# Sweethyh/GaussianImage_plus

Hardware: AMD Instinct MI355X
Metric: training iters/sec (fwd+bwd rasterize) at N Gaussians, 768x512 (higher is better)
Workload: dtype f32

## Files before the change

gaussianimage_plus_amd/csrc/gi2d_fused_core.h:

```cpp
#pragma once
#include <cstdint>

#include <hip/hip_runtime.h>

#ifdef GI2D_FUSED_TRACE
namespace gi2d {
__device__ unsigned long long *g_fused_trace = nullptr;
}
#define GI2D_TRACE_AT(wg, i)                                                                        \
    do {                                                                                            \
        if (threadIdx.x == 0 && g_fused_trace) g_fused_trace[(wg) * 16 + (i)] = wall_clock64();     \
    } while (0)
#define GI2D_TRACE(i) GI2D_TRACE_AT(tile, i)
#define GI2D_TRACE_VALUE(i, v)                                                        \
    do {                                                                              \
        if (threadIdx.x == 0 && g_fused_trace) g_fused_trace[tile * 16 + (i)] = (v);  \
    } while (0)
#define GI2D_BWD_TRACE(i) GI2D_TRACE_AT(blockIdx.x, i)
#define GI2D_HEAD_TRACE(i) GI2D_TRACE_AT(tile, i)
#else
#define GI2D_TRACE(i) \
    do {              \
    } while (0)
#define GI2D_TRACE_VALUE(i, v) \
    do {                       \
    } while (0)
#endif

#include "gi2d_fast_internal.h"

namespace gi2d {

#ifndef GI2D_FUSED_OCC
#define GI2D_FUSED_OCC 6
#endif

#ifndef GI2D_SMALL_CAP
#define GI2D_SMALL_CAP 128
#endif
template <int CAP>
struct FusedLdsT {
    static constexpr int PSTR = 9;
    static constexpr bool HAS_FIDX = false;
    static constexpr bool HAS_RAW = false;
    static constexpr int PART_ROWS = GI2D_BWD_PART_ROWS;
    static constexpr int LISTLEN = CAP + 8;
    static constexpr int IDS = CAP == GI2D_TILE_LIST_CAP ? GI2D_FAST_C : CAP;
    float4 gA[CAP + 1];
    float4 gB[CAP + 1];
    float2 gC[CAP + 2];
    unsigned cullw[CAP];
    float sse_w[4];
    int scan_w[8];
    int grp[32];
    union {
        struct {
            int ids[IDS];
        };
        struct {
            unsigned char lists[4][2 * LISTLEN];
            float4 pairbuf[GI2D_FWD_PAIRBUF];
        };
        struct {
            float4 pix[2 * GI2D_BWD_PIXRECS];
            unsigned short span[CAP];
            unsigned short item[8 * CAP];
            float part[GI2D_BWD_PART_ROWS * PSTR];
            int wsum[8];
            int n_items;
        };
        struct {
            char fwd_reach[sizeof(unsigned char) * 4 * 2 * LISTLEN + sizeof(float4) * GI2D_FWD_PAIRBUF];
            int slot[CAP];
        };
    };
    __device__ __forceinline__ void set_box(int, unsigned) {}
    __device__ __forceinline__ unsigned box_of(int k) const { return cullw[k] >> 8; }
};
typedef FusedLdsT<GI2D_TILE_LIST_CAP> FusedLds;
typedef FusedLdsT<GI2D_SMALL_CAP> FusedLdsSmall;
#ifndef GI2D_SMALL_OCC
#define GI2D_SMALL_OCC 8
#endif

static_assert(GI2D_FUSED_OCC < 6 || sizeof(FusedLds) <= 26624,
              "FusedLds: the sixth workgroup per CU needs <= 26 KB (see GI2D_FUSED_OCC)");
static_assert(sizeof(FusedLdsSmall) <= 160 * 1024 / GI2D_SMALL_OCC - 512, "FusedLdsSmall: eight workgroups per CU need <= 19.5 KB");
static_assert(offsetof(FusedLds, slot) >= offsetof(FusedLds, part) &&
                  offsetof(FusedLds, slot) + sizeof(int) * GI2D_TILE_LIST_CAP <= offsetof(FusedLds, wsum),
              "FusedLds: the partial-row codes must overlay the hand-off buffer only");
static_assert(offsetof(FusedLdsSmall, slot) >= offsetof(FusedLdsSmall, part) &&
                  offsetof(FusedLdsSmall, slot) + sizeof(int) * GI2D_SMALL_CAP <= offsetof(FusedLdsSmall, wsum),
              "FusedLdsSmall: the partial-row codes must overlay the hand-off buffer only");

template <int MODE, int CAP = GI2D_TILE_LIST_CAP, int FWD_UNROLL = GI2D_FWD_UNROLL, bool INBOX = false, bool WT = false>
__device__ __forceinline__ void fused_tile(
    FusedLdsT<CAP> &sm, int tile, int tiles_x, int tiles_y, int img_w, int img_h, const float4 *__restrict__ recs,
    int32_t *__restrict__ lists, int2 *__restrict__ tile_bins,
    float4 *__restrict__ partial_g, float4 *__restrict__ partial_big, int32_t *__restrict__ status,
    float *__restrict__ out_img, const float *__restrict__ vsrc, float grad_scale, float *__restrict__ tile_sse,
    const HeadRow head_row, const Inbox &ib) {
    const int tx = tile % tiles_x, ty = tile / tiles_x;
    const int pool_rows = tiles_x * tiles_y * GI2D_TILE_LIST_CAP;
    static_assert(CAP <= GI2D_TILE_LIST_CAP, "at most the reference's 256 entries of a tile are rasterized");
    const int tid = threadIdx.x, lane = tid & 63, wv = tid >> 6;
    const int lx = fwd_lane_col(tid), ly = tid >> 4;
    const int j = tx * GI2D_TILE + lx, i = ty * GI2D_TILE + ly;
    const bool inside = (i < img_h) && (j < img_w);
    const size_t pix = (size_t)i * img_w + j;

    GI2D_TRACE(0);
    float p0 = 0.f, p1 = 0.f, p2 = 0.f;
    if (inside) {
        p0 = vsrc[3 * pix];
        p1 = vsrc[3 * pix + 1];
        p2 = vsrc[3 * pix + 2];
    }

    if (tid == 0) {
        sm.gA[CAP] = make_float4(0.f, 0.f, 0.f, 0.f);
        sm.gB[CAP] = make_float4(0.f, 0.f, 0.f, 0.f);
        sm.gC[CAP] = make_float2(0.f, 0.f);
    }
    GI2D_TRACE_VALUE(1, (unsigned long long)blockIdx.x);
    const float tx0 = (float)(tx * GI2D_TILE), ty0 = (float)(ty * GI2D_TILE);
// ... 113 lines not shown
```

gaussianimage_plus_amd/csrc/gi2d_raster_core.h:

```cpp
#pragma once
#include "gi2d_common.h"

namespace gi2d {

#define GI2D_ALPHA_MIN (1.f / 255.f)
typedef float v2f __attribute__((ext_vector_type(2)));

struct GaussRec {
    float gx, gy, a, b;
    float c, opac, cr, cg;
    float cb;
    int slot;
    int gid;
    int pad;
};
static_assert(sizeof(GaussRec) == 48, "GaussRec must be 3 x float4");

__device__ __forceinline__ GaussRec load_gaussian(int g, const float2 *__restrict__ xys,
                                                  const float *__restrict__ conics,
                                                  const float *__restrict__ colors,
                                                  const float *__restrict__ opacities) {
    GaussRec r;
    const float2 xy = xys[g];
    r.gx = xy.x;
// ... 274 lines not shown
    if (background_fill) {
        o0 = background[0];
        o1 = background[1];
        o2 = background[2];
        cur_idx = 0;
    }
    if (inside) {
        const int pix = i * img_w + j;
        if (final_Ts) final_Ts[pix] = 1.f;
        if (NEED_FIDX) final_idx[pix] = cur_idx;
    }
    if (WT && (img_w & 3) == 0 && (reinterpret_cast<uintptr_t>(out_img) & 15) == 0 && (tx + 1) * GI2D_TILE <= img_w &&
        (ty + 1) * GI2D_TILE <= img_h)
        fwd_store_pixels_wt(o0, o1, o2, tx, ty, img_w, mybuf, out_img);
    else
        fwd_store_pixels(o0, o1, o2, tx, ty, img_w, img_h, out_img);
}

#ifndef GI2D_BWD_ITEMS
#define GI2D_BWD_ITEMS 256
#endif
static_assert(GI2D_BWD_ITEMS == 256, "an item's row in the hand-off buffer is its lane");
#ifndef GI2D_BWD_PART_ROWS
#define GI2D_BWD_PART_ROWS 176
#endif
#ifndef GI2D_BWD_OCC
#define GI2D_BWD_OCC 5
#endif

template <int PSTR, bool WT = false>
__device__ __forceinline__ void store_partial_row(float4 *__restrict__ dst, const float (&acc)[PSTR], int tag,
                                                  const void *wt_base = nullptr);

#define GI2D_BWD_PIXRECS (GI2D_TILE / 2 * GI2D_TILE)

template <bool WITH_ABS, bool FIDX = true>
struct BwdLds {
    static constexpr int PSTR = WITH_ABS ? 11 : 9;
    static constexpr bool HAS_FIDX = FIDX;
    static constexpr bool HAS_RAW = WITH_ABS;
    float4 pix[2 * GI2D_BWD_PIXRECS];
    float4 gA[GI2D_TILE_LIST_CAP];
    float4 gB[GI2D_TILE_LIST_CAP];
    float2 gC[GI2D_TILE_LIST_CAP];
    float4 gRaw[WITH_ABS ? GI2D_TILE_LIST_CAP : 1];
    unsigned short span[GI2D_TILE_LIST_CAP];
    unsigned short item[8 * GI2D_TILE_LIST_CAP];
    static constexpr int PART_ROWS = GI2D_BWD_PART_ROWS;
    float part[PART_ROWS * PSTR];
    unsigned xr[GI2D_TILE_LIST_CAP];
    int wsum[8];
    int n_items;
    __device__ __forceinline__ void set_box(int k, unsigned cull) { xr[k] = cull >> 8; }
    __device__ __forceinline__ unsigned box_of(int k) const { return xr[k]; }
};

template <class Lds>
__device__ __forceinline__ void bwd_publish_pixel(Lds &sm, int lx, int ly, float vx, float vy, float vz, float fi) {
    float *r = reinterpret_cast<float *>(&sm.pix[2 * ((ly >> 1) * GI2D_TILE + lx)]) + (ly & 1);
    r[0] = vx;
    r[2] = vy;
    r[4] = vz;
    if (Lds::HAS_FIDX) r[6] = fi;
}
template <class Lds>
__device__ __forceinline__ void bwd_stage_pixels(Lds &sm, int tx, int ty, int img_w, int img_h,
                                                 const int32_t *__restrict__ final_idx,
                                                 const float *__restrict__ v_output) {
    const int tid = threadIdx.x;
    const int lx = tid & 15, ly = tid >> 4;
    const int j = tx * GI2D_TILE + lx, i = ty * GI2D_TILE + ly;
    float vx = 0.f, vy = 0.f, vz = 0.f, fi = __int_as_float(-1);
    if (i < img_h && j < img_w) {
        const size_t pix = (size_t)i * img_w + j;
        vx = v_output[3 * pix];
        vy = v_output[3 * pix + 1];
        vz = v_output[3 * pix + 2];
        if (Lds::HAS_FIDX) fi = __int_as_float(final_idx ? final_idx[pix] : 0x7fffffff);
    }
    bwd_publish_pixel(sm, lx, ly, vx, vy, vz, fi);
}

template <class Lds>
__device__ __forceinline__ void bwd_stage_entry(Lds &sm, int k, const GaussRec &r, unsigned lim) {
    const ConicS s = scale_conic(r.a, r.b, r.c);
    sm.gA[k] = make_float4(r.gx, r.gy, s.ha, s.hb);
    sm.gB[k] = make_float4(s.hc, r.opac, r.cr, r.cg);
    sm.gC[k] = make_float2(r.cb, __int_as_float((int)lim));
    if constexpr (Lds::HAS_RAW) sm.gRaw[k] = make_float4(r.a, r.b, r.c, 0.f);
}

#ifndef GI2D_BWD_TRACE
#define GI2D_BWD_TRACE(i) \
    do {                  \
    } while (0)
#endif
// ... 16 lines not shown
    return it;
}
__device__ __forceinline__ unsigned long long bwd_prescan(int *wsum, unsigned cull) {
    if (__ballot((cull & 15u) != 0u) == 0ull) {
        if ((threadIdx.x & 63) == 63) wsum[2 * (threadIdx.x >> 6)] = 0, wsum[2 * (threadIdx.x >> 6) + 1] = 0;
        return 0ull;
    }
    const unsigned long long c = bwd_items_of(cull).counts;
    const unsigned lo = (unsigned)wave_inclusive_scan((int)(unsigned)c);
    const unsigned hi = (unsigned)wave_inclusive_scan((int)(unsigned)(c >> 32));
    if ((threadIdx.x & 63) == 63) wsum[2 * (threadIdx.x >> 6)] = (int)lo, wsum[2 * (threadIdx.x >> 6) + 1] = (int)hi;
    return (unsigned long long)hi << 32 | lo;
}
__device__ __forceinline__ int bwd_field_sum(unsigned long long packed) {
    return (int)((packed & 0xffffu) + ((packed >> 16) & 0xffffu) + ((packed >> 32) & 0xffffu) + (packed >> 48));
}

template <bool USE_FIDX>
__device__ __forceinline__ bool fidx_admits(int idx, float fidx_bits) {
    return !USE_FIDX || idx <= __float_as_int(fidx_bits);
}

struct BwdItemAcc {
    v2f S0, S1, S2, gr, gg, gb, ax, ay;
};
struct BwdItemIn {
    float gx, px0;
    v2f dy, bdy, cdy2;
    v2f ha2, opac2, cr2, cg2, cb2;
    float4 raw;
    unsigned lim_a, lim_b;
    int idx;
    const float4 *rec, *rec_end;
};
template <bool WITH_ABS, bool USE_FIDX, bool CLAMP>
__device__ __forceinline__ void bwd_item_columns(const BwdItemIn &in, BwdItemAcc &o) {
    const float4 *rec = in.rec;
    float px = in.px0;
#pragma unroll 1
    do {
        const float4 P0 = rec[0];
        float4 P1;
        if (USE_FIDX) {
            P1 = rec[1];
        } else {
            const float2 h = *reinterpret_cast<const float2 *>(rec + 1);
            P1 = make_float4(h.x, h.y, 0.f, 0.f);
        }
        const v2f vox = {P0.x, P0.y}, voy = {P0.z, P0.w}, voz = {P1.x, P1.y};
        const float dx1 = in.gx - px;
        px += 1.f;
        const v2f dx = {dx1, dx1};
        const v2f sig = __builtin_elementwise_fma(dx, __builtin_elementwise_fma(in.ha2, dx, in.bdy), in.cdy2);
        const v2f vis = {pair_vis(sig.x), pair_vis(sig.y)};
        const v2f t = in.opac2 * vis;
        const bool l0 = CLAMP ? pair_lands_odd(sig.x, t.x, in.lim_a) : pair_lands(sig.x, in.lim_a);
        const bool l1 = CLAMP ? pair_lands_odd(sig.y, t.y, in.lim_b) : pair_lands(sig.y, in.lim_b);
        const bool ok0 = fidx_admits<USE_FIDX>(in.idx, P1.z) & l0;
        const bool ok1 = fidx_admits<USE_FIDX>(in.idx, P1.w) & l1;
        const v2f tz = {ok0 ? t.x : 0.f, ok1 ? t.y : 0.f};
        v2f am = tz;
        if (CLAMP) am = (v2f){fminf(1.f, tz.x), fminf(1.f, tz.y)};
        const v2f v_alpha =
            __builtin_elementwise_fma(in.cb2, voz, __builtin_elementwise_fma(in.cg2, voy, in.cr2 * vox));
        o.gr = __builtin_elementwise_fma(am, vox, o.gr);
        o.gg = __builtin_elementwise_fma(am, voy, o.gg);
        o.gb = __builtin_elementwise_fma(am, voz, o.gb);
        const v2f w = tz * v_alpha;
        o.S0 += w;
        const v2f wdx = w * dx;
        o.S1 += wdx;
        o.S2 = __builtin_elementwise_fma(wdx, dx, o.S2);
        if (WITH_ABS) {
            const v2f a2 = {in.raw.x, in.raw.x}, b2 = {in.raw.y, in.raw.y}, c2 = {in.raw.z, in.raw.z};
            const v2f ux = w * __builtin_elementwise_fma(a2, dx, b2 * in.dy);
            const v2f uy = w * __builtin_elementwise_fma(b2, dx, c2 * in.dy);
            o.ax += __builtin_elementwise_abs(ux);
            o.ay += __builtin_elementwise_abs(uy);
        }
        rec += 2;
    } while (rec <= in.rec_end);
}

template <bool WITH_ABS, bool USE_FIDX = true, bool PRESCANNED = false, bool WT = false, class Lds = BwdLds<WITH_ABS, USE_FIDX>>
__device__ __forceinline__ void bwd_run_tile(Lds &sm, int len, unsigned cull, int list_base, float tx0, float ty0,
                                             float4 *__restrict__ dst, unsigned long long prescan_incl = 0ull,
                                             const int *prescan_wsum = nullptr, const void *wt_base = nullptr) {
    constexpr int PSTR = Lds::PSTR;
    static_assert(!USE_FIDX || Lds::HAS_FIDX, "final_idx is not staged in this LDS layout");
    static_assert(!WITH_ABS || Lds::HAS_RAW, "the |v_xy| sums need the conic as given");
    const int tid = threadIdx.x, wv = tid >> 6;
    unsigned long long incl = prescan_incl;
    const int *wsum = prescan_wsum;
    if (!PRESCANNED) {
        incl = bwd_prescan(sm.wsum, cull);
        wsum = sm.wsum;
        __syncthreads();
    }
    const bool placing = (tid & ~63) < len || wv == 0;
    if (placing) {
        unsigned long long before = 0ull, total = 0ull;
#pragma unroll
        for (int k = 0; k < 4; ++k) {
            const unsigned lo = (unsigned)__builtin_amdgcn_readfirstlane(wsum[2 * k]);
            const unsigned hi = (unsigned)__builtin_amdgcn_readfirstlane(wsum[2 * k + 1]);
            const unsigned long long w = (unsigned long long)hi << 32 | lo;
            total += w;
            if (k < __builtin_amdgcn_readfirstlane(wv)) before += w;
        }
        const unsigned long long class_base = (total << 16) + (total << 32) + (total << 48);
        const BwdItemsOf mine = bwd_items_of(cull);
        const unsigned long long pos = before + class_base + (incl - mine.counts);
        const int slot0 = (int)((pos >> (16 * mine.cls)) & 0xffffu);
// ... 31 lines not shown
    }

    int round0 = 0;
    do {
        const int round1 = min(n_items, round0 + GI2D_BWD_ITEMS);
        const int it = round0 + tid;
        float res[PSTR];
        if (it < round1) {
            const int code = sm.item[it], k = code & 255;
            const unsigned xr = sm.box_of(k);
            const int r0 = (int)(xr & 15u), r1 = (int)((xr >> 4) & 15u);
            const int p = (r0 >> 1) + (code >> 8);
            const int c_lo = (int)((xr >> 8) & 15u);
            const int c_hi = (int)((xr >> 12) & 15u);
            const float4 A = sm.gA[k], B = sm.gB[k];
            const float2 C = sm.gC[k];
            BwdItemIn in;
            const bool in_a = 2 * p >= r0, in_b = 2 * p + 1 <= r1;
            in.gx = A.x;
            const float gy = A.y;
            ConicS s;
            s.ha = A.z, s.hb = A.w, s.hc = B.x;
            const float py_a = ty0 + (float)(2 * p);
            in.dy = (v2f){gy - py_a, gy - (py_a + 1.f)};
            in.bdy = (v2f){row_term_b(s, in.dy.x), row_term_b(s, in.dy.y)};
            in.cdy2 = (v2f){row_term_c(s, in.dy.x), row_term_c(s, in.dy.y)};
            in.ha2 = (v2f){s.ha, s.ha}, in.opac2 = (v2f){B.y, B.y};
            in.cr2 = (v2f){B.z, B.z}, in.cg2 = (v2f){B.w, B.w}, in.cb2 = (v2f){C.x, C.x};
            in.lim_a = in_a ? (unsigned)__float_as_int(C.y) : 0u;
            in.lim_b = in_b ? (unsigned)__float_as_int(C.y) : 0u;
            in.idx = list_base + k;
            in.raw = make_float4(0.f, 0.f, 0.f, 0.f);
            if constexpr (WITH_ABS) in.raw = sm.gRaw[k];
            in.rec = &sm.pix[2 * (p * GI2D_TILE + c_lo)];
            in.rec_end = in.rec + 2 * (c_hi - c_lo);
            in.px0 = tx0 + (float)c_lo;
            const v2f zero2 = {0.f, 0.f};
            BwdItemAcc o;
            o.S0 = o.S1 = o.S2 = o.gr = o.gg = o.gb = o.ax = o.ay = zero2;
            if (__ballot((xr >> 16) & 1u) != 0ull)
                bwd_item_columns<WITH_ABS, USE_FIDX, true>(in, o);
            else
                bwd_item_columns<WITH_ABS, USE_FIDX, false>(in, o);
            const v2f dy = in.dy, S0 = o.S0, S1 = o.S1, S2 = o.S2, gr = o.gr, gg = o.gg, gb = o.gb, ax = o.ax, ay = o.ay;
            const float u0a = dy.x * S0.x, u0b = dy.y * S0.y;
            res[0] = S1.x + S1.y;
            res[1] = u0a + u0b;
            res[2] = S2.x + S2.y;
            res[3] = __builtin_fmaf(dy.x, S1.x, dy.y * S1.y);
            res[4] = __builtin_fmaf(dy.x, u0a, dy.y * u0b);
            res[5] = gr.x + gr.y;
            res[6] = gg.x + gg.y;
            res[7] = gb.x + gb.y;
            res[8] = S0.x + S0.y;
            if (WITH_ABS) {
                res[PSTR - 2] = ax.x + ax.y;
                res[PSTR - 1] = ay.x + ay.y;
            }
        }
        GI2D_BWD_TRACE(8);
#if defined(GI2D_STOP_AFTER) && GI2D_STOP_AFTER == 5
        if (n_items >= 0) {
            float all = 0.f;
#pragma unroll
            for (int q = 0; q < PSTR; ++q) all += res[q];
            if (it < round1 && all == 12345.678f) sm.part[0] = all;
            return;
        }
#endif
        constexpr int PROWS = Lds::PART_ROWS;
        const int lo = max(my_lo, round0), hi = min(my_hi, round1);
        const bool owner = dst != nullptr && (hi > lo || (round0 == 0 && my_hi == my_lo));
        float acc[PSTR];
#pragma unroll
        for (int q = 0; q < PSTR; ++q) acc[q] = 0.f;
#pragma unroll
// ... 105 lines not shown
```

gaussianimage_plus_amd/csrc/gi2d_capi.hip:

```cpp
#include <string>

#include "gi2d_common.h"

namespace gi2d {

static thread_local std::string g_last_error;

void set_error(const char *msg) { g_last_error = msg ? msg : ""; }

int check_launch(const char *what) {
    const hipError_t e = hipGetLastError();
    if (e == hipSuccess) return GI2D_OK;
    g_last_error = std::string(what) + ": " + hipGetErrorString(e);
    return (int)e;
}

#define GI2D_STR2(x) #x
#define GI2D_STR(x) GI2D_STR2(x)
static std::string dev_switches() {
    std::string s;
    const auto add = [&](const char *name, const char *value) {
        if (!s.empty()) s += ' ';
        s += name;
        if (value && *value) s += std::string("=") + value;
    };
    (void)add;
#ifdef GI2D_STOP_AFTER
    add("GI2D_STOP_AFTER", GI2D_STR(GI2D_STOP_AFTER));
#endif
#ifdef GI2D_FUSED_TRACE
    add("GI2D_FUSED_TRACE", "");
#endif
#ifdef GI2D_UPDATE_STOP
    add("GI2D_UPDATE_STOP", GI2D_STR(GI2D_UPDATE_STOP));
#endif
#ifdef GI2D_INBOX_STATS
    add("GI2D_INBOX_STATS", "");
#endif
#ifdef GI2D_DEV_VARIANT
    add("GI2D_DEV_VARIANT", GI2D_STR(GI2D_DEV_VARIANT));
#endif
    return s;
}

}

extern "C" {
const char *gi2d_version(void) {
    static const std::string v = [] {
        std::string s = "gi2d 0.3.0 (gfx950)";
        const std::string d = gi2d::dev_switches();
        if (!d.empty()) s += " dev[" + d + "]";
        return s;
    }();
    return v.c_str();
}
const char *gi2d_last_error_string(void) { return gi2d::g_last_error.c_str(); }
}
```

gaussianimage_plus_amd/csrc/gi2d_fast.hip:

```cpp
#include <cstdio>
#include <cstdlib>
#include <cstring>
#include <mutex>
#include <unordered_map>
#include <vector>

#include <hip/hip_ext.h>

#include "gi2d_fused_core.h"
#include "gi2d_batch.h"

namespace gi2d {

__global__ __launch_bounds__(256) void fast_fill_kernel(int n, const float2 *__restrict__ xys,
                                                        const int32_t *__restrict__ radii,
                                                        const float *__restrict__ conics,
                                                        const float *__restrict__ colors,
                                                        const float *__restrict__ opacities, int tiles_x, int tiles_y,
                                                        float radius_clip, PrevBox *__restrict__ prev_box,
                                                        int32_t *__restrict__ lists, RecSets rs,
                                                        int32_t *__restrict__ status) {
    const int g = blockIdx.x * blockDim.x + threadIdx.x;
    begin_binning(g, status);
    const BinRecs recs = recs_for_binning(rs, g == 0);
// ... 313 lines not shown
__global__ __launch_bounds__(256) void fast_reduce_kernel(
    int n, const PrevBox *__restrict__ prev_box, int tiles_x, int tiles_y, const int32_t *__restrict__ gids_sorted,
    const int2 *__restrict__ tile_bins, const float4 *__restrict__ partial_g, const float4 *__restrict__ partial_big,
    float2 *__restrict__ v_xy, float *__restrict__ v_conic, float *__restrict__ v_rgb, float *__restrict__ v_opacity,
    float4 *__restrict__ v_abs_xy) {
    const int g = blockIdx.x * blockDim.x + threadIdx.x;
    float acc[11];
    const PrevBox pb = g < n ? prev_box[g] : no_box();
    reduce_one(g, make_int2(pb.x, pb.y), pb.z, tiles_x * tiles_y * GI2D_TILE_LIST_CAP, partial_g, partial_big, acc);
    if (g < n) store_grads(g, acc, v_xy, v_conic, v_rgb, v_opacity, v_abs_xy);
}

struct NextProject {
    float clip_coe;
    const float2 *means2d;
    float *depths;
    int32_t *num_tiles_hit;
    BinTarget bt;
    int32_t *tile_order;
};

template <int KIND, bool FILL_NEXT>
__global__ __launch_bounds__(256) void fast_reduce_project_kernel(
    int n, int role_blocks, float2 *xys, int32_t *radii, float *conics, int tiles_x, int tiles_y, float radius_clip,
    PrevBox *prev_box, const int32_t *__restrict__ gids_sorted, const int2 *__restrict__ tile_bins,
    const float4 *__restrict__ partial_g, const float4 *__restrict__ partial_big, const float *__restrict__ p0,
    const float *__restrict__ p1, float img_w, float img_h, float2 *__restrict__ v_xy, float *__restrict__ v_conic,
    float *__restrict__ v_rgb, float *__restrict__ v_opacity, float4 *__restrict__ v_abs_xy,
    float *__restrict__ v_cov2d, float2 *__restrict__ v_mean2d, float *__restrict__ v_p0, float *__restrict__ v_p1,
    NextProject next) {
    int block = blockIdx.x;
    if (FILL_NEXT) {
        if (block >= 2 * role_blocks) {
            compute_tile_order(tile_bins, tiles_x * tiles_y, next.tile_order);
            return;
        }
        if (block >= role_blocks) {
            project_fill_one<KIND>((block - role_blocks) * blockDim.x + threadIdx.x, n, next.clip_coe, next.means2d, p0,
                                   p1, img_w, img_h, tiles_x, tiles_y, radius_clip, xys, next.depths, radii, conics,
                                   next.num_tiles_hit, next.bt);
            return;
        }
    }
    const int g = block * blockDim.x + threadIdx.x;
    int2 box = make_int2(0, 0);
    int pool = -1;
    float conic[3] = {0.f, 0.f, 0.f};
    int radius = 0;
    if (g < n) {
        if (FILL_NEXT) {
            const float4 *rec = recs_of_last_pass(next.bt.recs) + 4 * (size_t)g;
            const float4 q0 = rec[0], q1 = rec[1], q2 = rec[2], q3 = rec[3];
            conic[0] = q0.z, conic[1] = q0.w, conic[2] = q1.x;
            box = make_int2(__float_as_int(q2.w), __float_as_int(q3.x));
            radius = __float_as_int(q3.y);
            pool = __float_as_int(q3.z);
        } else {
            const PrevBox pb = prev_box[g];
            box = make_int2(pb.x, pb.y), pool = pb.z;
            conic[0] = conics[3 * g], conic[1] = conics[3 * g + 1], conic[2] = conics[3 * g + 2];
            radius = radii[g];
        }
    }
    float par[3] = {0.f, 0.f, 0.f};
    if (g < n) {
        if (KIND == kScaleRot)
            par[0] = p0[2 * g], par[1] = p0[2 * g + 1], par[2] = p1[g];
// ... 663 lines not shown
```

gaussianimage_plus_amd/csrc/gi2d_fast_internal.h:

```cpp
#pragma once
#include <atomic>
#include <type_traits>

#include "gi2d_project_core.h"
#include "gi2d_raster_core.h"

namespace gi2d {


#define GI2D_FAST_C 1024
#define GI2D_FAST_HDR 16
#define GI2D_INBOX_WORDS 64
#define GI2D_INBOX_SLOTS (32 * GI2D_INBOX_WORDS)
#define GI2D_INBOX_MAX_TILES 1536
#define GI2D_FAST_LROW (GI2D_FAST_C + GI2D_FAST_HDR + GI2D_INBOX_WORDS)
#define GI2D_FAST_EPT (GI2D_FAST_C / 256)
#define GI2D_FAST_S 32
#ifndef GI2D_FILL_BATCH
#define GI2D_FILL_BATCH 16
#endif
#ifndef GI2D_REDUCE_BATCH
#define GI2D_REDUCE_BATCH 8
#endif
#define GI2D_BIG_TILES_F 32
// ... 416 lines not shown
}
template <bool INBOX = false, class Between>
__device__ __forceinline__ void bin_projected(int g, const ProjOut &o, float opac, float cr, float cg, float cb,
                                              int tiles_x, int tiles_y, float radius_clip, PrevBox old_box,
                                              PrevBox *__restrict__ prev_box, int32_t *__restrict__ lists,
                                              const BinRecs &recs, Between between, InboxFill *in = nullptr) {
    bin_one<INBOX>(g, o.xy, o.radius, o.tiles_hit > 0, o.k0, o.k1, o.k2, opac, cr, cg, cb, tiles_x, tiles_y, radius_clip,
                   old_box, prev_box, lists, recs, between, in);
}
__device__ __forceinline__ void bin_projected(int g, const ProjOut &o, float opac, float cr, float cg, float cb,
                                              int tiles_x, int tiles_y, float radius_clip, PrevBox old_box,
                                              PrevBox *__restrict__ prev_box, int32_t *__restrict__ lists,
                                              const BinRecs &recs) {
    bin_projected(g, o, opac, cr, cg, cb, tiles_x, tiles_y, radius_clip, old_box, prev_box, lists, recs, [] {});
}

__device__ __forceinline__ int partial_slot(int g, int2 box, int tx, int ty, int pool) {
    int mnx, mny, mxx, mxy;
    unpack_box(box, mnx, mny, mxx, mxy);
    const int w = mxx - mnx, ntiles = w * (mxy - mny), at = (ty - mny) * w + (tx - mnx);
    if (ntiles <= GI2D_FAST_S) return g * GI2D_FAST_S + at;
    return -(pool + at) - 1;
}
__device__ __forceinline__ float4 *partial_row(int slot, float4 *__restrict__ partial_g, float4 *__restrict__ partial_big,
                                               int pool_rows, int32_t *__restrict__ status) {
    if (slot >= 0) return partial_g + GI2D_FAST_ROW * (size_t)slot;
    const int row = -slot - 1;
    if (row < 0 || row >= pool_rows) {
        atomicOr(&status[1], GI2D_STATUS_POOL);
        atomicOr(&status[2], GI2D_STATUS_POOL);
        return nullptr;
    }
    return partial_big + GI2D_FAST_ROW * (size_t)row;
}

#ifndef GI2D_HEAD_TRACE
#define GI2D_HEAD_TRACE(i) \
    do {                   \
    } while (0)
#endif
struct HeadRow {
    int hdr_count, hdr_sorted, id0;
    unsigned inbox_w;
};
__device__ __forceinline__ HeadRow head_row_load(const int32_t *__restrict__ lists, int tile, bool inbox) {
    const int32_t *row = lists + (size_t)tile * GI2D_FAST_LROW;
    HeadRow h;
    h.hdr_count = row[0], h.hdr_sorted = row[1], h.id0 = row[GI2D_FAST_HDR + threadIdx.x];
    h.inbox_w = 0u;
    if (inbox) h.inbox_w = (unsigned)row[GI2D_FAST_HDR + GI2D_FAST_C + (threadIdx.x & 63)];
    return h;
}
__device__ __forceinline__ HeadRow head_row_for(const int32_t *__restrict__ lists, const int32_t *__restrict__ order,
                                                int slot, int &tile, bool inbox) {
    HeadRow h = head_row_load(lists, slot, inbox);
    tile = __builtin_amdgcn_readfirstlane(order[slot]);
    if (tile != slot) h = head_row_load(lists, tile, inbox);
    return h;
}
template <bool OPTIMISTIC, int EPT, bool INBOX, class Prep, class Put>
__device__ __forceinline__ int tile_list_head_rows(int *ids, int *grp, int tile, int tx, int ty,
                                                   const float4 *__restrict__ recs, int32_t *__restrict__ row,
                                                   int2 *__restrict__ tile_bins, int32_t *__restrict__ status, Prep prep,
                                                   Put put, int id0, int hdr_count, int hdr_sorted, int count, int sorted,
                                                   unsigned inbox_w, const float4 *__restrict__ inbox) {
    const int tid = threadIdx.x, lane = tid & 63, wv = tid >> 6;
// ... 180 lines not shown
            }
            const unsigned long long km = __ballot(keep);
            const int len = __popcll(km);
            int rank = lane;
            if (!(len == count && sorted == count)) {
                ids[lane] = keep ? g : -1;
                __builtin_amdgcn_wave_barrier();
                rank = 0;
                for (int q = 0; q < count; ++q) rank += ((unsigned)ids[q] < (unsigned)g) ? 1 : 0;
                const bool in_place = lane < sorted && rank == lane;
                if (keep && !in_place) row[GI2D_FAST_HDR + rank] = g;
            }
            if (keep) put(rank, g, prep(g, r0));
            if (lane == 0) {
                if (hdr_count != len || hdr_sorted != len) {
                    row[0] = len;
                    row[1] = len;
                }
                tile_bins[tile] = make_int2(list_base(tile), list_base(tile) + len);
                grp[0] = len;
            }
        }
        __syncthreads();
        return grp[0];
    }
    if (count <= 256)
        return tile_list_head_rows<OPTIMISTIC, 1, INBOX>(ids, grp, tile, tx, ty, recs, row, tile_bins, status, prep, put, hr.id0,
                                                  hdr_count, hdr_sorted, count, sorted, hr.inbox_w, inbox);
    return tile_list_head_rows<OPTIMISTIC, GI2D_FAST_EPT, INBOX>(ids, grp, tile, tx, ty, recs, row, tile_bins, status, prep, put,
                                                          hr.id0, hdr_count, hdr_sorted, count, sorted, hr.inbox_w, inbox);
}

#define GI2D_ORDER_BINS (GI2D_FAST_C + 1)
#define GI2D_CU_SLOTS 256
#define GI2D_ORDER_MAX_TILES 2048
__device__ __forceinline__ void compute_tile_order(const int2 *__restrict__ tile_bins, int num_tiles,
                                                   int32_t *__restrict__ tile_order, bool always = false) {
    if (num_tiles <= GI2D_CU_SLOTS || num_tiles > GI2D_ORDER_MAX_TILES) return;
    __shared__ int hist[GI2D_ORDER_BINS + 1];
    const int tid = threadIdx.x, bs = blockDim.x;
    for (int b = tid; b <= GI2D_ORDER_BINS; b += bs) hist[b] = 0;
    constexpr int PL = GI2D_ORDER_MAX_TILES / 64;
    int pop[PL];
    int2 rr[PL];
#pragma unroll
    for (int q = 0; q < PL; ++q) rr[q] = tile_bins[min(tid + q * bs, num_tiles - 1)];
#pragma unroll
    for (int q = 0; q < PL; ++q) pop[q] = tid + q * bs < num_tiles ? min(max(rr[q].y - rr[q].x, 0), GI2D_ORDER_BINS - 1) : 0;
    {
        __shared__ int red_max[4], red_sum[4];
        int mx = 0, sm = 0;
#pragma unroll
        for (int q = 0; q < PL; ++q) mx = max(mx, pop[q]), sm += pop[q];
#pragma unroll
        for (int d = 32; d >= 1; d >>= 1) mx = max(mx, __shfl_xor(mx, d, 64)), sm += __shfl_xor(sm, d, 64);
        if ((tid & 63) == 0) red_max[tid >> 6] = mx, red_sum[tid >> 6] = sm;
        __syncthreads();
        mx = 0, sm = 0;
        for (int k = 0; k < (bs >> 6); ++k) mx = max(mx, red_max[k]), sm += red_sum[k];
        if (!always && 4 * mx * num_tiles <= 7 * sm) return;
    }
    __syncthreads();
#pragma unroll
    for (int q = 0; q < PL; ++q)
        if (tid + q * bs < num_tiles) atomicAdd(&hist[GI2D_ORDER_BINS - 1 - pop[q]], 1);
    __syncthreads();
    if (tid < 64) {
        constexpr int PER = (GI2D_ORDER_BINS + 63) / 64;
        int v[PER], sum = 0;
#pragma unroll
        for (int q = 0; q < PER; ++q) {
            const int b = tid * PER + q;
            v[q] = b < GI2D_ORDER_BINS ? hist[b] : 0;
            sum += v[q];
        }
        int run = wave_inclusive_scan(sum) - sum;
#pragma unroll
        for (int q = 0; q < PER; ++q) {
            const int b = tid * PER + q;
            if (b < GI2D_ORDER_BINS) hist[b] = run;
            run += v[q];
        }
    }
    __syncthreads();
    const int full_rounds = num_tiles / GI2D_CU_SLOTS;
#pragma unroll
    for (int q = 0; q < PL; ++q) {
        const int t = tid + q * bs;
        if (t >= num_tiles) continue;
        const int rank = atomicAdd(&hist[GI2D_ORDER_BINS - 1 - pop[q]], 1);
        const int round = rank / GI2D_CU_SLOTS, pos = rank % GI2D_CU_SLOTS;
        const int slot = (round < full_rounds && (round & 1)) ? GI2D_CU_SLOTS - 1 - pos : pos;
        tile_order[round * GI2D_CU_SLOTS + slot] = t;
    }
}
// ... 81 lines not shown
```

gaussianimage_plus_amd/csrc/gi2d_train.hip:

```cpp
#include <cstring>
#include <vector>

#include "gi2d_batch.h"
#include "gi2d_quant_core.h"

namespace gi2d {

__device__ __forceinline__ int live_n(const TrainParams &P, int n) { return P.n_dev ? min(n, *P.n_dev) : n; }

struct __attribute__((may_alias)) Row3 {
    float a, b, c;
};
struct __attribute__((may_alias, aligned(8))) Row2 {
    float x, y;
};
__device__ __forceinline__ Row3 load_row3(const float *p, int g) { return *reinterpret_cast<const Row3 *>(p + 3 * (size_t)g); }
__device__ __forceinline__ void store_row3(float *p, int g, float a, float b, float c) {
    Row3 r;
    r.a = a, r.b = b, r.c = c;
    *reinterpret_cast<Row3 *>(p + 3 * (size_t)g) = r;
}
__device__ __forceinline__ float2 load_row2(const float *p, int g) {
    const Row2 r = reinterpret_cast<const Row2 *>(p)[g];
    return make_float2(r.x, r.y);
// ... 222 lines not shown
        } else {
            float s0, s1, s2, s3;
            if (c.parallel) {
                __shared__ float chunk_s[4];
                const float mine = chunk_sum(wv, true);
                if (lane == 0) chunk_s[wv] = mine;
                __syncthreads();
                s0 = chunk_s[0], s1 = chunk_s[1], s2 = chunk_s[2], s3 = chunk_s[3];
            } else {
                s0 = chunk_sum(0, true), s1 = chunk_sum(1, false), s2 = chunk_sum(2, false), s3 = chunk_sum(3, false);
            }
            total = (s0 + s1) + (s2 + s3);
        }
        const float prev = best.sse[best.step & 1];
        snapshot = total < prev;
        if (g == 0) {
            best.sse[(best.step + 1) & 1] = snapshot ? total : prev;
            if (snapshot) {
                best.info[0] = n;
                best.info[1] = best.step;
            }
        }
    }
    return snapshot;
}

template <int KIND, bool FILL_NEXT, bool ADAN, bool INBOX = false, bool ALONE = INBOX>
__device__ __forceinline__ void train_reduce_update_body(int block, bool order_block, const UpdateArgs &u,
                                                         const AdamStep &a_xyz, const AdamStep &a_chol,
                                                         const AdamStep &a_feat, int step) {
#pragma clang fp contract(off)
    const int tiles_x = u.tiles_x, tiles_y = u.tiles_y;
    if (order_block) {
        if ((step & 15) == 1) compute_tile_order(u.tile_bins, tiles_x * tiles_y, u.next.tile_order, true);
        return;
    }
    const TrainParams &P = u.P;
    const NextFill &next = u.next;
    const PrevBox *prev_box = u.next.prev_box;
    float2 *xys = u.xys;
    int32_t *radii = u.radii;
    float *conics = u.conics;
    const float img_w = u.img_w, img_h = u.img_h, radius_clip = u.radius_clip;
    float *dbg_grads = u.dbg_grads;
    BestSnap best = u.best;
    best.step = step;
    const int g = block * blockDim.x + threadIdx.x;
    const bool in_rows = g < u.n;
    AdamRows rows;
    if (!ADAN && in_rows) rows = adam_load_rows(P, g);
    const PrevBox box_ld = in_rows ? prev_box[g] : no_box();
    const int radius = in_rows ? radii[g] : 0;
    float conic[3] = {0.f, 0.f, 0.f};
    if (in_rows) conic[0] = conics[3 * g], conic[1] = conics[3 * g + 1], conic[2] = conics[3 * g + 2];
    const float opac_next = (FILL_NEXT && in_rows) ? P.opacity[g] : 0.f;
    constexpr int AHEAD = ALONE ? GI2D_UPDATE_ROWS_AHEAD : 0;
    const RowsAhead<AHEAD> ahead = rows_ahead<AHEAD>(u.partial_g, in_rows ? g : 0);
    const Row3 bound_row = in_rows ? load_row3(P.bound, P.bound_stride ? g : 0) : Row3{0.f, 0.f, 0.f};
    const float bound3[3] = {bound_row.a, bound_row.b, bound_row.c};
    const int n = live_n(P, u.n);
    const PrevBox pbox = g < n ? box_ld : no_box();
    const int2 box = make_int2(pbox.x, pbox.y);
    const SseLoads sse_first = best_sse_loads(best);
    const bool snapshot = best_decision(best, sse_first, n, g);
    float acc[11];
    InboxFill inbox;
    reduce_one<AHEAD>(g, box, pbox.z, tiles_x * u.tiles_y * GI2D_TILE_LIST_CAP, u.partial_g, u.partial_big,
// ... 1341 lines not shown
```

Measured before the change: 37230.

## Split backward pixel LDS records into padded planar arrays

Splits the interleaved backward pixel staging buffer into two arrays: a float4 array holding the x/y values and a separate float2 (or float4 when final_idx is staged) array for the z value. The row pitch is padded by one column, presumably to reduce LDS bank conflicts when items walk columns. This also avoids loading unused padding in the no-final_idx case. In exchange the padding makes the LDS footprint slightly larger, the part buffer is moved after wsum/n_items, and the overlay static asserts are relaxed, which could affect occupancy limits or aliasing.

Result: no change. 37350 (median of 6 runs) (+0.3%).

```diff
diff --git a/gaussianimage_plus_amd/csrc/gi2d_fused_core.h b/gaussianimage_plus_amd/csrc/gi2d_fused_core.h
--- a/gaussianimage_plus_amd/csrc/gi2d_fused_core.h
+++ b/gaussianimage_plus_amd/csrc/gi2d_fused_core.h
@@ -44,6 +44,7 @@
     static constexpr bool HAS_FIDX = false;
     static constexpr bool HAS_RAW = false;
     static constexpr int PART_ROWS = GI2D_BWD_PART_ROWS;
+    typedef float2 PixZ;
     static constexpr int LISTLEN = CAP + 8;
     static constexpr int IDS = CAP == GI2D_TILE_LIST_CAP ? GI2D_FAST_C : CAP;
     float4 gA[CAP + 1];
@@ -62,12 +63,13 @@
             float4 pairbuf[GI2D_FWD_PAIRBUF];
         };
         struct {
-            float4 pix[2 * GI2D_BWD_PIXRECS];
+            float4 pixA[GI2D_BWD_PIXRECS];
+            float2 pixZ[GI2D_BWD_PIXRECS];
             unsigned short span[CAP];
             unsigned short item[8 * CAP];
-            float part[GI2D_BWD_PART_ROWS * PSTR];
             int wsum[8];
             int n_items;
+            float part[GI2D_BWD_PART_ROWS * PSTR];
         };
         struct {
             char fwd_reach[sizeof(unsigned char) * 4 * 2 * LISTLEN + sizeof(float4) * GI2D_FWD_PAIRBUF];
@@ -86,11 +88,12 @@
 static_assert(GI2D_FUSED_OCC < 6 || sizeof(FusedLds) <= 26624,
               "FusedLds: the sixth workgroup per CU needs <= 26 KB (see GI2D_FUSED_OCC)");
 static_assert(sizeof(FusedLdsSmall) <= 160 * 1024 / GI2D_SMALL_OCC - 512, "FusedLdsSmall: eight workgroups per CU need <= 19.5 KB");
-static_assert(offsetof(FusedLds, slot) >= offsetof(FusedLds, part) &&
-                  offsetof(FusedLds, slot) + sizeof(int) * GI2D_TILE_LIST_CAP <= offsetof(FusedLds, wsum),
+static_assert(offsetof(FusedLds, slot) >= offsetof(FusedLds, part) && offsetof(FusedLds, part) > offsetof(FusedLds, n_items) &&
+                  offsetof(FusedLds, part) > offsetof(FusedLds, wsum),
               "FusedLds: the partial-row codes must overlay the hand-off buffer only");
 static_assert(offsetof(FusedLdsSmall, slot) >= offsetof(FusedLdsSmall, part) &&
-                  offsetof(FusedLdsSmall, slot) + sizeof(int) * GI2D_SMALL_CAP <= offsetof(FusedLdsSmall, wsum),
+                  offsetof(FusedLdsSmall, part) > offsetof(FusedLdsSmall, n_items) &&
+                  offsetof(FusedLdsSmall, part) > offsetof(FusedLdsSmall, wsum),
               "FusedLdsSmall: the partial-row codes must overlay the hand-off buffer only");
 
 template <int MODE, int CAP = GI2D_TILE_LIST_CAP, int FWD_UNROLL = GI2D_FWD_UNROLL, bool INBOX = false, bool WT = false>
diff --git a/gaussianimage_plus_amd/csrc/gi2d_raster_core.h b/gaussianimage_plus_amd/csrc/gi2d_raster_core.h
--- a/gaussianimage_plus_amd/csrc/gi2d_raster_core.h
+++ b/gaussianimage_plus_amd/csrc/gi2d_raster_core.h
@@ -330,14 +330,25 @@
 __device__ __forceinline__ void store_partial_row(float4 *__restrict__ dst, const float (&acc)[PSTR], int tag,
                                                   const void *wt_base = nullptr);
 
-#define GI2D_BWD_PIXRECS (GI2D_TILE / 2 * GI2D_TILE)
+#define GI2D_BWD_PIXPITCH (GI2D_TILE + 1)
+#define GI2D_BWD_PIXRECS (GI2D_TILE / 2 * GI2D_BWD_PIXPITCH)
+template <bool FIDX>
+struct BwdPixZ {
+    typedef float4 type;
+};
+template <>
+struct BwdPixZ<false> {
+    typedef float2 type;
+};
 
 template <bool WITH_ABS, bool FIDX = true>
 struct BwdLds {
     static constexpr int PSTR = WITH_ABS ? 11 : 9;
     static constexpr bool HAS_FIDX = FIDX;
     static constexpr bool HAS_RAW = WITH_ABS;
-    float4 pix[2 * GI2D_BWD_PIXRECS];
+    typedef typename BwdPixZ<FIDX>::type PixZ;
+    float4 pixA[GI2D_BWD_PIXRECS];
+    PixZ pixZ[GI2D_BWD_PIXRECS];
     float4 gA[GI2D_TILE_LIST_CAP];
     float4 gB[GI2D_TILE_LIST_CAP];
     float2 gC[GI2D_TILE_LIST_CAP];
@@ -355,11 +366,12 @@
 
 template <class Lds>
 __device__ __forceinline__ void bwd_publish_pixel(Lds &sm, int lx, int ly, float vx, float vy, float vz, float fi) {
-    float *r = reinterpret_cast<float *>(&sm.pix[2 * ((ly >> 1) * GI2D_TILE + lx)]) + (ly & 1);
-    r[0] = vx;
-    r[2] = vy;
-    r[4] = vz;
-    if (Lds::HAS_FIDX) r[6] = fi;
+    const int at = (ly >> 1) * GI2D_BWD_PIXPITCH + lx;
+    float *ra = reinterpret_cast<float *>(&sm.pixA[at]) + (ly & 1), *rz = reinterpret_cast<float *>(&sm.pixZ[at]) + (ly & 1);
+    ra[0] = vx;
+    ra[2] = vy;
+    rz[0] = vz;
+    if constexpr (Lds::HAS_FIDX) rz[2] = fi;
 }
 template <class Lds>
 __device__ __forceinline__ void bwd_stage_pixels(Lds &sm, int tx, int ty, int img_w, int img_h,
@@ -442,21 +454,20 @@
     unsigned lim_a, lim_b;
     int idx;
     const float4 *rec, *rec_end;
-};
-template <bool WITH_ABS, bool USE_FIDX, bool CLAMP>
+    const void *rec_z;
+};
+template <bool WITH_ABS, bool USE_FIDX, bool CLAMP, class PixZ>
 __device__ __forceinline__ void bwd_item_columns(const BwdItemIn &in, BwdItemAcc &o) {
+    static_assert(!USE_FIDX || sizeof(PixZ) == sizeof(float4), "final_idx is not staged in this LDS layout");
     const float4 *rec = in.rec;
+    const PixZ *rec_z = static_cast<const PixZ *>(in.rec_z);
     float px = in.px0;
 #pragma unroll 1
     do {
-        const float4 P0 = rec[0];
-        float4 P1;
-        if (USE_FIDX) {
-            P1 = rec[1];
-        } else {
-            const float2 h = *reinterpret_cast<const float2 *>(rec + 1);
-            P1 = make_float4(h.x, h.y, 0.f, 0.f);
-        }
+        const float4 P0 = *rec;
+        const PixZ h = *rec_z;
+        float4 P1 = make_float4(h.x, h.y, 0.f, 0.f);
+        if constexpr (USE_FIDX) P1 = h;
         const v2f vox = {P0.x, P0.y}, voy = {P0.z, P0.w}, voz = {P1.x, P1.y};
         const float dx1 = in.gx - px;
         px += 1.f;
@@ -488,7 +499,7 @@
             o.ax += __builtin_elementwise_abs(ux);
             o.ay += __builtin_elementwise_abs(uy);
         }
-        rec += 2;
+        ++rec, ++rec_z;
     } while (rec <= in.rec_end);
 }
 
@@ -586,16 +597,17 @@
             in.idx = list_base + k;
             in.raw = make_float4(0.f, 0.f, 0.f, 0.f);
             if constexpr (WITH_ABS) in.raw = sm.gRaw[k];
-            in.rec = &sm.pix[2 * (p * GI2D_TILE + c_lo)];
-            in.rec_end = in.rec + 2 * (c_hi - c_lo);
+            in.rec = &sm.pixA[p * GI2D_BWD_PIXPITCH + c_lo];
+            in.rec_end = in.rec + (c_hi - c_lo);
+            in.rec_z = &sm.pixZ[p * GI2D_BWD_PIXPITCH + c_lo];
             in.px0 = tx0 + (float)c_lo;
             const v2f zero2 = {0.f, 0.f};
             BwdItemAcc o;
             o.S0 = o.S1 = o.S2 = o.gr = o.gg = o.gb = o.ax = o.ay = zero2;
             if (__ballot((xr >> 16) & 1u) != 0ull)
-                bwd_item_columns<WITH_ABS, USE_FIDX, true>(in, o);
+                bwd_item_columns<WITH_ABS, USE_FIDX, true, typename Lds::PixZ>(in, o);
             else
-                bwd_item_columns<WITH_ABS, USE_FIDX, false>(in, o);
+                bwd_item_columns<WITH_ABS, USE_FIDX, false, typename Lds::PixZ>(in, o);
             const v2f dy = in.dy, S0 = o.S0, S1 = o.S1, S2 = o.S2, gr = o.gr, gg = o.gg, gb = o.gb, ax = o.ax, ay = o.ay;
             const float u0a = dy.x * S0.x, u0b = dy.y * S0.y;
             res[0] = S1.x + S1.y;
```

## Order tiles by XCD-local spatial blocks for L2 locality in raster scheduling

Applied to the files above, without the earlier changes.

Extends the tile-order computation so that, when the tile count is a multiple of 256, tiles are grouped into eight spatial blocks, one per XCD, and sorted by workload within each block. Tiles are then interleaved so that round-robin block dispatch places neighbouring tiles on the same XCD. The goal is better L2 reuse of shared Gaussian data while keeping load balance. If one block is much heavier than the rest, it falls back to a global workload sort with serpentine slots. The cost is a larger shared histogram and more index arithmetic, though this step only runs every 16th training step.

Result: faster. 36730 before, 37310 after (median of 6 runs) (+1.6%).

```diff
diff --git a/gaussianimage_plus_amd/csrc/gi2d_capi.hip b/gaussianimage_plus_amd/csrc/gi2d_capi.hip
--- a/gaussianimage_plus_amd/csrc/gi2d_capi.hip
+++ b/gaussianimage_plus_amd/csrc/gi2d_capi.hip
@@ -37,6 +37,9 @@
 #ifdef GI2D_INBOX_STATS
     add("GI2D_INBOX_STATS", "");
 #endif
+#ifdef GI2D_XCD_ORDER
+    add("GI2D_XCD_ORDER", GI2D_STR(GI2D_XCD_ORDER));
+#endif
 #ifdef GI2D_DEV_VARIANT
     add("GI2D_DEV_VARIANT", GI2D_STR(GI2D_DEV_VARIANT));
 #endif
diff --git a/gaussianimage_plus_amd/csrc/gi2d_fast.hip b/gaussianimage_plus_amd/csrc/gi2d_fast.hip
--- a/gaussianimage_plus_amd/csrc/gi2d_fast.hip
+++ b/gaussianimage_plus_amd/csrc/gi2d_fast.hip
@@ -369,7 +369,7 @@
     int block = blockIdx.x;
     if (FILL_NEXT) {
         if (block >= 2 * role_blocks) {
-            compute_tile_order(tile_bins, tiles_x * tiles_y, next.tile_order);
+            compute_tile_order(tile_bins, tiles_x, tiles_y, next.tile_order);
             return;
         }
         if (block >= role_blocks) {
diff --git a/gaussianimage_plus_amd/csrc/gi2d_fast_internal.h b/gaussianimage_plus_amd/csrc/gi2d_fast_internal.h
--- a/gaussianimage_plus_amd/csrc/gi2d_fast_internal.h
+++ b/gaussianimage_plus_amd/csrc/gi2d_fast_internal.h
@@ -472,6 +472,40 @@
         return nullptr;
     }
     return partial_big + GI2D_FAST_ROW * (size_t)row;
+}
+
+#define GI2D_CU_SLOTS 256
+#define GI2D_ORDER_MAX_TILES 2048
+#ifndef GI2D_XCD_ORDER
+#define GI2D_XCD_ORDER 1
+#endif
+#define GI2D_XCDS 8
+__host__ __device__ __forceinline__ bool xcd_order_applies(int num_tiles) {
+    return GI2D_XCD_ORDER != 0 && num_tiles > GI2D_CU_SLOTS && num_tiles <= GI2D_ORDER_MAX_TILES &&
+           num_tiles % GI2D_CU_SLOTS == 0;
+}
+__host__ __device__ __forceinline__ int small_div(int x, float inv) { return (int)(((float)x + 0.5f) * inv); }
+struct XcdBlocks {
+    int shift;
+    int bw, bh;
+    float inv_bw, inv_bh, inv_tx;
+};
+__host__ __device__ __forceinline__ XcdBlocks xcd_blocks(int tiles_x, int tiles_y) {
+    int best = 0, cost = 0x7fffffff;
+#pragma unroll
+    for (int s = 0; s <= 3; ++s) {
+        const int c = (tiles_x >> s) + (tiles_y >> (3 - s));
+        if ((tiles_x & ((1 << s) - 1)) == 0 && (tiles_y & ((8 >> s) - 1)) == 0 && c < cost) cost = c, best = s;
+    }
+    XcdBlocks b;
+    b.shift = best;
+    b.bw = tiles_x >> best, b.bh = tiles_y >> (3 - best);
+    b.inv_bw = 1.f / (float)b.bw, b.inv_bh = 1.f / (float)b.bh, b.inv_tx = 1.f / (float)tiles_x;
+    return b;
+}
+__host__ __device__ __forceinline__ int xcd_block_of_tile(const XcdBlocks &b, int tile, int tiles_x) {
+    const int ty = small_div(tile, b.inv_tx), tx = tile - ty * tiles_x;
+    return (small_div(ty, b.inv_bh) << b.shift) + small_div(tx, b.inv_bw);
 }
 
 #ifndef GI2D_HEAD_TRACE
@@ -718,14 +752,17 @@
 }
 
 #define GI2D_ORDER_BINS (GI2D_FAST_C + 1)
-#define GI2D_CU_SLOTS 256
-#define GI2D_ORDER_MAX_TILES 2048
-__device__ __forceinline__ void compute_tile_order(const int2 *__restrict__ tile_bins, int num_tiles,
+#define GI2D_ORDER_XBINS 256
+static_assert(GI2D_XCDS * GI2D_ORDER_XBINS == GI2D_ORDER_MAX_TILES && GI2D_ORDER_MAX_TILES % 64 == 0, "one histogram, 32 bins per lane of the scanning wave");
+__device__ __forceinline__ void compute_tile_order(const int2 *__restrict__ tile_bins, int tiles_x, int tiles_y,
                                                    int32_t *__restrict__ tile_order, bool always = false) {
+    const int num_tiles = tiles_x * tiles_y;
     if (num_tiles <= GI2D_CU_SLOTS || num_tiles > GI2D_ORDER_MAX_TILES) return;
-    __shared__ int hist[GI2D_ORDER_BINS + 1];
+    constexpr int HIST = GI2D_XCD_ORDER ? GI2D_ORDER_MAX_TILES : GI2D_ORDER_BINS + 1;
+    __shared__ int hist[HIST >= GI2D_ORDER_BINS + 1 ? HIST : GI2D_ORDER_BINS + 1];
     const int tid = threadIdx.x, bs = blockDim.x;
-    for (int b = tid; b <= GI2D_ORDER_BINS; b += bs) hist[b] = 0;
+    const bool xcd = xcd_order_applies(num_tiles);
+    for (int b = tid; b < (int)(sizeof(hist) / sizeof(int)); b += bs) hist[b] = 0;
     constexpr int PL = GI2D_ORDER_MAX_TILES / 64;
     int pop[PL];
     int2 rr[PL];
@@ -733,8 +770,8 @@
     for (int q = 0; q < PL; ++q) rr[q] = tile_bins[min(tid + q * bs, num_tiles - 1)];
 #pragma unroll
     for (int q = 0; q < PL; ++q) pop[q] = tid + q * bs < num_tiles ? min(max(rr[q].y - rr[q].x, 0), GI2D_ORDER_BINS - 1) : 0;
+    __shared__ int red_max[4], red_sum[4];
     {
-        __shared__ int red_max[4], red_sum[4];
         int mx = 0, sm = 0;
 #pragma unroll
         for (int q = 0; q < PL; ++q) mx = max(mx, pop[q]), sm += pop[q];
@@ -747,6 +784,67 @@
         if (!always && 4 * mx * num_tiles <= 7 * sm) return;
     }
     __syncthreads();
+    if (GI2D_XCD_ORDER && xcd) {
+        const XcdBlocks xb = xcd_blocks(tiles_x, tiles_y);
+#pragma unroll
+        for (int q = 0; q < PL; ++q) {
+            const int t = tid + q * bs;
+            if (t >= num_tiles) continue;
+            pop[q] = xcd_block_of_tile(xb, t, tiles_x) * GI2D_ORDER_XBINS + (GI2D_ORDER_XBINS - 1 - (min(pop[q], 1023) >> 2));
+            atomicAdd(&hist[pop[q]], 1);
+        }
+        __syncthreads();
+        __shared__ int by_block;
+        if (tid < 64) {
+            constexpr int PER = GI2D_ORDER_MAX_TILES / 64;
+            int sum = 0, wsum = 0;
+#pragma unroll 8
+            for (int q = 0; q < PER; ++q) {
+                const int i = tid * PER + q, c = hist[i];
+                sum += c;
+                wsum += c * (4 * (GI2D_ORDER_XBINS - 1 - (i & (GI2D_ORDER_XBINS - 1))) + 2);
+            }
+#pragma unroll
+            for (int d = 1; d <= 4; d <<= 1) wsum += __shfl_xor(wsum, d, 64);
+            int heaviest = wsum, all = wsum;
+#pragma unroll
+            for (int d = 8; d <= 32; d <<= 1) heaviest = max(heaviest, __shfl_xor(heaviest, d, 64)), all += __shfl_xor(all, d, 64);
+            const bool local = 16 * GI2D_XCDS * heaviest <= 17 * all;
+            const auto at = [&](int i) { return local ? i : (i & (GI2D_XCDS - 1)) * GI2D_ORDER_XBINS + (i >> 3); };
+            if (!local) {
+                sum = 0;
+#pragma unroll 8
+                for (int q = 0; q < PER; ++q) sum += hist[at(tid * PER + q)];
+            }
+            int run = wave_inclusive_scan(sum) - sum;
+#pragma unroll 8
+            for (int q = 0; q < PER; ++q) {
+                const int i = at(tid * PER + q), c = hist[i];
+                hist[i] = run;
+                run += c;
+            }
+            if (tid == 0) by_block = local ? 1 : 0;
+        }
+        __syncthreads();
+        const bool local = by_block != 0;
+        const int per_block = num_tiles / GI2D_XCDS, full_rounds = num_tiles / GI2D_CU_SLOTS;
+#pragma unroll
+        for (int q = 0; q < PL; ++q) {
+            const int t = tid + q * bs;
+            if (t >= num_tiles) continue;
+            const int rank = atomicAdd(&hist[pop[q]], 1);
+            if (local) {
+                const int x = pop[q] / GI2D_ORDER_XBINS, r = rank - x * per_block;
+                const int round = r >> 5, pos = r & 31;
+                tile_order[round * GI2D_CU_SLOTS + ((round & 1) ? 31 - pos : pos) * GI2D_XCDS + x] = t;
+            } else {
+                const int round = rank / GI2D_CU_SLOTS, pos = rank % GI2D_CU_SLOTS;
+                const int slot = (round < full_rounds && (round & 1)) ? GI2D_CU_SLOTS - 1 - pos : pos;
+                tile_order[round * GI2D_CU_SLOTS + slot] = t;
+            }
+        }
+        return;
+    }
 #pragma unroll
     for (int q = 0; q < PL; ++q)
         if (tid + q * bs < num_tiles) atomicAdd(&hist[GI2D_ORDER_BINS - 1 - pop[q]], 1);
diff --git a/gaussianimage_plus_amd/csrc/gi2d_train.hip b/gaussianimage_plus_amd/csrc/gi2d_train.hip
--- a/gaussianimage_plus_amd/csrc/gi2d_train.hip
+++ b/gaussianimage_plus_amd/csrc/gi2d_train.hip
@@ -278,7 +278,7 @@
 #pragma clang fp contract(off)
     const int tiles_x = u.tiles_x, tiles_y = u.tiles_y;
     if (order_block) {
-        if ((step & 15) == 1) compute_tile_order(u.tile_bins, tiles_x * tiles_y, u.next.tile_order, true);
+        if ((step & 15) == 1) compute_tile_order(u.tile_bins, tiles_x, tiles_y, u.next.tile_order, true);
         return;
     }
     const TrainParams &P = u.P;
```
